# jilljenn/TF-recomm

Measured on AMD Instinct MI355X. Metric: training ratings/sec + val RMSE, MovieLens-1M SVD dim=64 @1 GPU, higher is better.
Workload: dtype f32

## Files before the change

### include/tfrecomm.h

```cpp
#ifndef TFRECOMM_H
#define TFRECOMM_H

#include <stdint.h>

#ifdef __cplusplus
extern "C" {
#endif

#define TFR_ABI_VERSION 3

typedef struct tfr_model tfr_model;

typedef enum {
    TFR_OK = 0,
    TFR_ERR_ARG = -1,
    TFR_ERR_OOB = -2,
    TFR_ERR_HIP = -3,
    TFR_ERR_STATE = -4,
    TFR_ERR_NOMEM = -5
} tfr_status;

enum {
    TFR_MU = 0,
    TFR_BU = 1,
// ... 233 lines not shown
int tfr_neighbours_dev(tfr_model* m, int32_t which, int32_t metric, const int32_t* d_rows, int64_t n, int32_t k,
                       const int64_t* d_excl_indptr, const int32_t* d_excl, int64_t lo, int64_t hi,
                       int32_t* d_ids_out, float* d_scores_out);
int tfr_svdpp_neighbours(tfr_svdpp* m, int32_t which, int32_t metric, const int32_t* rows, int64_t n, int32_t k,
                         const int64_t* excl_indptr, const int32_t* excl, int64_t lo, int64_t hi,
                         int32_t* ids_out, float* scores_out);
int tfr_svdpp_neighbours_dev(tfr_svdpp* m, int32_t which, int32_t metric, const int32_t* d_rows, int64_t n, int32_t k,
                             const int64_t* d_excl_indptr, const int32_t* d_excl, int64_t lo, int64_t hi,
                             int32_t* d_ids_out, float* d_scores_out);
int tfr_fm_neighbours(tfr_fm* m, int32_t metric, const int32_t* features, int64_t n, int32_t k,
                      const int64_t* excl_indptr, const int32_t* excl, int64_t lo, int64_t hi,
                      int32_t* ids_out, float* scores_out);
int tfr_neighbours_plan(int32_t dim, int32_t k, int64_t n, int64_t n_candidates,
                        int64_t* lds_bytes, int32_t* rows_per_block, int32_t* slices, int64_t* row_chunk);

enum {
    TFR_K_FORWARD = 0,
    TFR_K_SORT = 1,
    TFR_K_REDUCE_ITEM = 2,
    TFR_K_REDUCE_USER = 3,
    TFR_K_APPLY = 4,
    TFR_K_FINALIZE = 5,
    TFR_K_GATHER = 6,
    TFR_K_DRAW = 7,
    TFR_K_COUNT = 8
};
int tfr_profile(tfr_model* m, int32_t enable);
int tfr_kernel_plan(tfr_model* m, int64_t batch, char* buf, int64_t buflen);
int tfr_profile_read(tfr_model* m, int32_t kernel, double* total_ms, int64_t* launches);

int tfr_lds_bytes(int32_t kernel, int32_t dim, int64_t batch, int64_t user_num, int64_t item_num,
                  int64_t* static_bytes, int64_t* dynamic_bytes);

int tfr_sync(tfr_model* m);
const char* tfr_last_error(void);
int tfr_version(void);
int tfr_device_count(void);
int tfr_device_copy_rate(int32_t device, int64_t bytes, int32_t reps, double* best_gbs, double* mean_gbs);

#ifdef __cplusplus
}
#endif
#endif
```

### tf-recomm_amd/_lib.py

```python
from __future__ import annotations

import ctypes as C
import os

import numpy as np

_HERE = os.path.dirname(os.path.abspath(__file__))
LIB_PATH = os.path.join(_HERE, "csrc", "libtfrecomm_hip.so")

ABI_VERSION = 3
OK, ERR_ARG, ERR_OOB, ERR_HIP, ERR_STATE, ERR_NOMEM = 0, -1, -2, -3, -4, -5
MU, BU, BI, P, Q = 0, 1, 2, 3, 4
Y = 5
SLOT_M, SLOT_V = 8, 16
LOSS = {"mse": 0, "nll": 1}
OPTIMIZER = {"adam": 0, "sgd": 1}
ADAM_MODE = {"tf1": 0, "lazy": 1}
K_FORWARD, K_SORT, K_REDUCE_ITEM, K_REDUCE_USER, K_APPLY, K_FINALIZE, K_GATHER, K_DRAW = range(8)
NB_ITEMS, NB_USERS = 0, 1
NB_METRIC = {"dot": 0, "cosine": 1}
KERNEL_NAMES = ["forward", "sort", "reduce_item", "reduce_user", "apply", "finalize", "gather", "draw"]


class TfrOpts(C.Structure):
# ... 83 lines not shown
    "tfr_staged_ids_devptr": (C.c_int, [_p, C.POINTER(_p), _i64p]),
    "tfr_fm_create": (C.c_int, [C.POINTER(_p), C.c_int64, C.c_int32, C.POINTER(TfrOpts)]),
    "tfr_fm_destroy": (C.c_int, [_p]),
    "tfr_fm_set": (C.c_int, [_p, C.c_float, _f32p, _f32p]),
    "tfr_fm_get": (C.c_int, [_p, _f32p, _f32p, _f32p]),
    "tfr_fm_get_table": (C.c_int, [_p, C.c_int32, _f32p, C.c_int64]),
    "tfr_fm_get_step": (C.c_int, [_p, _i64p, _f32p, _f32p]),
    "tfr_fm_train_step": (C.c_int, [_p, _i64p, _i32p, _f32p, _f32p, C.c_int64, _f32p, _f32p]),
    "tfr_fm_train_step_dev": (C.c_int, [_p, _p, _p, _p, _p, C.c_int64, C.c_int64, _p]),
    "tfr_fm_init": (C.c_int, [_p, C.c_uint64, C.c_float]),
    "tfr_fm_forward": (C.c_int, [_p, _i64p, _i32p, _f32p, C.c_int64, _f32p]),
    "tfr_fm_forward_dev": (C.c_int, [_p, _p, _p, _p, C.c_int64, _p]),
    "tfr_fm_sync": (C.c_int, [_p, _f32p]),
    "tfr_fm_last_error": (C.c_char_p, []),
    "tfr_fm_upload_rows": (C.c_int, [_p, C.c_int32, _i64p, _i32p, _f32p, _f32p, C.c_int64]),
    "tfr_fm_train_steps_resident": (C.c_int, [_p, _i64p, C.c_int64, C.c_int32, _f32p]),
    "tfr_fm_gather_rows": (C.c_int, [_p, C.c_int32, _i64p, C.c_int64, _i64p, _i32p, _f32p, _f32p, C.c_int64]),
    "tfr_fm_predict_resident": (C.c_int, [_p, C.c_int32, _f32p]),
    "tfr_fm_eval_binary_resident": (C.c_int, [_p, _i64p, _f64p, _f64p, _i64p]),
    "tfr_als_create": (C.c_int, [C.POINTER(_p), C.c_int64, C.c_int64, C.c_int32, C.c_double, C.c_int32]),
    "tfr_als_destroy": (C.c_int, [_p]),
    "tfr_als_set": (C.c_int, [_p, _f64p, _f64p, _f64p, _f64p]),
    "tfr_als_get": (C.c_int, [_p, _f64p, _f64p, _f64p, _f64p, _f64p]),
    "tfr_als_set_bias": (C.c_int, [_p, C.c_double]),
    "tfr_als_load": (C.c_int, [_p, _i64p, _i64p, _f64p, C.c_int64]),
    "tfr_als_sweep": (C.c_int, [_p, C.c_int32, _f32p]),
    "tfr_als_predict": (C.c_int, [_p, _i64p, _i64p, C.c_int64, _f64p]),
    "tfr_als_last_error": (C.c_char_p, []),
    "tfr_sort_segments": (C.c_int, [_p, C.c_int32, _i32p, C.c_int64, _i32p, _i32p]),
    "tfr_kernel_plan": (C.c_int, [_p, C.c_int64, C.c_char_p, C.c_int64]),
    "tfr_profile": (C.c_int, [_p, C.c_int32]),
    "tfr_profile_read": (C.c_int, [_p, C.c_int32, C.POINTER(C.c_double), _i64p]),
    "tfr_lds_bytes": (C.c_int, [C.c_int32, C.c_int32, C.c_int64, C.c_int64, C.c_int64, _i64p, _i64p]),
    "tfr_topk": (C.c_int, [_p, _i32p, C.c_int64, C.c_int32, _i64p, _i32p, _i32p, _f32p]),
    "tfr_topk_dev": (C.c_int, [_p, _p, C.c_int64, C.c_int32, _p, _p, _p, _p]),
    "tfr_fm_topk": (C.c_int, [_p, _i32p, C.c_int64, C.c_int64, C.c_int64, C.c_int32, _i64p, _i32p, _i32p, _f32p]),
    "tfr_topk_plan": (C.c_int, [C.c_int32, C.c_int32, C.c_int64, C.c_int64, _i64p, _i32p, _i32p, _i64p]),
    "tfr_neighbours": (C.c_int, [_p, C.c_int32, C.c_int32, _i32p, C.c_int64, C.c_int32, _i64p, _i32p, C.c_int64, C.c_int64,
                                 _i32p, _f32p]),
    "tfr_neighbours_dev": (C.c_int, [_p, C.c_int32, C.c_int32, _p, C.c_int64, C.c_int32, _p, _p, C.c_int64, C.c_int64, _p, _p]),
    "tfr_svdpp_neighbours": (C.c_int, [_p, C.c_int32, C.c_int32, _i32p, C.c_int64, C.c_int32, _i64p, _i32p, C.c_int64,
                                       C.c_int64, _i32p, _f32p]),
    "tfr_svdpp_neighbours_dev": (C.c_int, [_p, C.c_int32, C.c_int32, _p, C.c_int64, C.c_int32, _p, _p, C.c_int64, C.c_int64,
                                           _p, _p]),
    "tfr_fm_neighbours": (C.c_int, [_p, C.c_int32, _i32p, C.c_int64, C.c_int32, _i64p, _i32p, C.c_int64, C.c_int64, _i32p,
                                    _f32p]),
    "tfr_neighbours_plan": (C.c_int, [C.c_int32, C.c_int32, C.c_int64, C.c_int64, _i64p, _i32p, _i32p, _i64p]),
    "tfr_rank_items": (C.c_int, [_p, _i32p, C.c_int64, _i64p, _i32p, _i64p, _i32p, _i32p]),
    "tfr_fm_rank_items": (C.c_int, [_p, _i32p, C.c_int64, C.c_int64, C.c_int64, _i64p, _i32p, _i64p, _i32p, _i32p]),
    "tfr_rank_plan": (C.c_int, [C.c_int32, C.c_int64, C.c_int64, C.c_int64, _i64p, _i32p, _i32p, _i32p, _i64p]),
    "tfr_finetune_users": (C.c_int, [_p, C.c_int64, _i32p, _i64p, _i32p, _f32p, _i64p, _i32p, _i32p, _i64p, C.c_int32,
                                     _f32p, _f32p, _f32p]),
    "tfr_finetune_plan": (C.c_int, [C.c_int32, C.c_int64, _i64p, _i32p, _i32p]),
    "tfr_svdpp_create": (C.c_int, [C.POINTER(_p), C.c_int64, C.c_int64, C.c_int32, C.POINTER(TfrOpts)]),
    "tfr_svdpp_destroy": (C.c_int, [_p]),
    "tfr_svdpp_set_table": (C.c_int, [_p, C.c_int32, _f32p, C.c_int64]),
    "tfr_svdpp_get_table": (C.c_int, [_p, C.c_int32, _f32p, C.c_int64]),
    "tfr_svdpp_init": (C.c_int, [_p, C.c_uint64, C.c_float, C.c_float]),
    "tfr_svdpp_set_implicit": (C.c_int, [_p, _i64p, _i32p]),
    "tfr_svdpp_set_frozen": (C.c_int, [_p, C.c_uint32]),
    "tfr_svdpp_set_hyper": (C.c_int, [_p, C.c_float, C.c_float]),
    "tfr_svdpp_get_step": (C.c_int, [_p, _i64p, _f32p, _f32p]),
    "tfr_svdpp_set_step": (C.c_int, [_p, C.c_int64, C.c_float, C.c_float]),
    "tfr_svdpp_forward": (C.c_int, [_p, _i32p, _i32p, C.c_int64, _f32p]),
    "tfr_svdpp_forward_dev": (C.c_int, [_p, _p, _p, C.c_int64, _p]),
    "tfr_svdpp_eval": (C.c_int, [_p, _i32p, _i32p, _f32p, C.c_int64, _f64p, _i64p]),
# ... 87 lines not shown
```

### tf-recomm_amd/csrc/api.hip

```cpp
#include <hip/hip_runtime.h>
#include <utility>
#include <stdarg.h>
#include <stdio.h>
#include <string.h>
#include <stdlib.h>
#include <math.h>
#include <new>
#include <chrono>
#include <vector>
#include <algorithm>
#include "tfrecomm.h"
#include "svd_kernels.h"
#include "topk.h"
#include "neighbours.h"
#include "rank.h"
#include "finetune.h"
#include "devbuf.h"

using namespace tfr;

static thread_local char g_err[512] = "";

static int fail(int code, const char* fmt, ...) {
    va_list ap;
// ... 2040 lines not shown

int tfr_lds_bytes(int32_t kernel, int32_t dim, int64_t batch, int64_t user_num, int64_t item_num,
                  int64_t* static_bytes, int64_t* dynamic_bytes) {
    int G, VEC;
    if (!geometry(dim, &G, &VEC)) return fail(TFR_ERR_ARG, "unsupported dim %d", dim);
    if (batch < 1 || user_num < 1 || item_num < 1) return fail(TFR_ERR_ARG, "lds_bytes: batch and row counts must be >= 1");
    const int bu = bits_for(user_num), bi = bits_for(item_num);
    const int nbmax = 1 << (bu > bi ? bu : bi);
    int64_t st = 0, dy = 0;
    if (kernel == 0 || kernel == 2) {
        if (nbmax > CSORT_MAX_BINS || !csort_eligible(batch, bu, bi)) return fail(TFR_ERR_ARG, "shape does not take the counting-sort path");
        const int64_t ntiles = (batch + CSORT_TILE - 1) / CSORT_TILE;
        if (kernel == 0) {
            if (ntiles > 16) return fail(TFR_ERR_ARG, "batch beyond 16 tiles does not take k_tile_step");
            const int epg = tile_step_epg((int)ntiles, G, VEC);
            st = (int64_t)tile_step_static_lds(G, epg);
            dy = (int64_t)tile_step_dyn_lds(G, VEC, epg, nbmax);
        } else {
            st = 256 * 4 + 16 * 64 * 4 + 16 * 3 * 4;
            dy = (int64_t)nbmax * 4;
        }
    } else if (kernel == 1 || kernel == 4) {
        st = (int64_t)seg_reduce_static_lds(G, VEC, kernel == 1);
    } else if (kernel == 3) {
        st = 2 * 624 * 4 + 2 * 10 * 4;
    } else {
        return fail(TFR_ERR_ARG, "lds_bytes: kernel must be 0 (k_tile_step), 1 (k_seg_reduce fwd), 2 (k_front), 3 (k_mt_draw), 4 (k_seg_reduce)");
    }
    if (static_bytes) *static_bytes = st;
    if (dynamic_bytes) *dynamic_bytes = dy;
    return TFR_OK;
}

static int ensure_ring(tfr_model* m, int64_t B) {
    if (B <= m->ring_cap) return TFR_OK;
    const int64_t cap = pow2_cap(B);
    m->ring_cap = 0;
    HIPCHK(m->d_ring.reserve(cap * tfr_model::HRING, m->stream));
    HIPCHK(m->h_ring.reserve(cap * tfr_model::HRING, m->stream));
    for (int z = 0; z < tfr_model::HRING; ++z)
        if (!m->ring_ev[z]) HIPCHK(hipEventCreateWithFlags(&m->ring_ev[z], hipEventDisableTiming));
    m->ring_cap = cap;
    return TFR_OK;
}

int tfr_train_step_ids(tfr_model* m, const int64_t* ids, int64_t B) {
    MODEL_ENTER(m);
    if (!m->N) return fail(TFR_ERR_STATE, "no resident triples: call tfr_upload_triples first");
    if (B < 1 || !ids) return fail(TFR_ERR_ARG, "bad batch / null ids");
    int rc;
    if ((rc = ensure_capacity(m, B))) return rc;
    if ((rc = ensure_ring(m, B))) return rc;
    const int z = m->ring_pos;
    m->ring_pos = (z + 1) % tfr_model::HRING;
    HIPCHK(hipEventSynchronize(m->ring_ev[z]));
    int64_t* h = m->h_ring + (size_t)z * m->ring_cap;
    int64_t* d = m->d_ring + (size_t)z * m->ring_cap;
    memcpy(h, ids, (size_t)B * 8);
    HIPCHK(hipMemcpyAsync(d, h, (size_t)B * 8, hipMemcpyHostToDevice, m->stream));
    HIPCHK(hipEventRecord(m->ring_ev[z], m->stream));
    m->pf_valid = false;
    return run_train_step(m, m->d_u, m->d_i, m->d_r, B, nullptr, nullptr, d, nullptr);
}

int tfr_forward_resident(tfr_model* m, int64_t lo, int64_t hi, float* logits_out) {
    MODEL_ENTER(m);
// ... 1227 lines not shown
```

### tf-recomm_amd/csrc/svd_kernels.h

```cpp
#pragma once
#include <hip/hip_runtime.h>
#include <stdint.h>

namespace tfr {

enum { MODE_INFER = 0, MODE_TRAIN = 1, MODE_EVAL = 2 };
enum { RMODE_SCRATCH = 0, RMODE_ADAM = 1, RMODE_SGD = 2 };


struct FwdArgs {
    const float* P; const float* Q; const float* bu; const float* bi; const float* mu;
    const int32_t* u; const int32_t* it; const float* r;
    const int64_t* ids; const int4* store;
    int32_t* u_out; int32_t* it_out;
    float* logits; float* g; float* partials; int32_t* err;
    int64_t B, U, I, N;
    int32_t D, loss, item_abs, reg_bias, lds_reduce;
    const int32_t* dB; int32_t qstride, bistride;
};

struct GatherArgs {
    const int64_t* ids;
    int64_t lo, B, N;
    const int4* store;
// ... 81 lines not shown
struct FinArgs {
    const float* partials; int32_t nblk;
    float* scalars; float* out;
    float* mu; float* mu_m; float* mu_v; const int32_t* err;
    int32_t update_mu, opt, clear_partials;
    int32_t out_err;
    float alpha, b1, b2, eps, lr;
};

struct ApplyPair { ApplyArgs a[2]; FinArgs f = {}; int32_t with_fin = 0; };

struct DenseArgs {
    int32_t* map; const int32_t* ks; const float* grad_rows; const float* grad_bias;
    float* dense_grad; float* dense_gbias;
    float* w; float* m; float* v; float* bias_w; float* bias_m; float* bias_v;
    const int32_t* err;
    int64_t rows, B;
    int32_t D, frozen_rows, frozen_bias, opt;
    float alpha, b1, b2, eps, lr;
};

struct DensePair { DenseArgs a[2]; FinArgs f; };


enum : int32_t {
    TFR_WT_ROWS = 1,
    TFR_WT_MOMENTS = 2,
    TFR_WT_BIAS = 4,
    TFR_WT_PIECES = 8,
    TFR_WT_PUBLISH = 16,
};
constexpr int32_t TFR_WT_DEFAULT = TFR_WT_ROWS | TFR_WT_MOMENTS | TFR_WT_BIAS | TFR_WT_PIECES | TFR_WT_PUBLISH;
int tile_step_wt();

struct TileDenseArgs {
    const int32_t* tab;
    const float* grad_rows; const float* grad_bias;
    float* w; float* m; float* v; float* bias_w; float* bias_m; float* bias_v;
    float* out_rows; float* out_bias;
    const int32_t* err;
    int64_t rows;
    int32_t D, nbins, ntiles, frozen_rows, frozen_bias, opt, skip_untouched;
    float alpha, b1, b2, eps, lr;
};
struct TileDenseLaunch { TileDenseArgs a[2]; FinArgs f; int32_t with_fin; int32_t wt; };
void launch_dense_tiles(const TileDenseLaunch& L, bool write, bool with_fin, int G, int VEC, hipStream_t s);

struct CSortArgs {
    const int32_t* keys[2];
    int32_t* ks[2]; int32_t* ps[2];
    int32_t* lrank[2];
    int32_t* hist[2];
    int32_t* offs[2];
    int32_t* binbase[2];
    int32_t* blocktot[2];
    int32_t nbins[2];
    int32_t ntiles;
    int64_t B;
};

struct FmArgs {
    const float* V; const float* W; const float* mu;
    const int64_t* indptr; const int32_t* indices; const float* data;
    float* out; int32_t* err;
    const float* y; float* s_rows; int4* ent; float* partials;
    int64_t n_rows, F;
    int32_t D, loss;
    float lam;
    int32_t variant;
};
int fm_grid(int64_t n_rows, int G, bool train);
void launch_fm(const FmArgs& a, bool train, int G, int VEC, int grid, hipStream_t s);

struct FrontArgs {
    FwdArgs f; CSortArgs c;
    int32_t* key_out[2];
    int32_t nfwd;
    int32_t tile_local;
};
// ... 131 lines not shown
```

### tf-recomm_amd/csrc/svd_kernels.hip

```cpp
#include <hip/hip_runtime.h>
#include <cstdlib>
#include <stdint.h>
#include "svd_kernels.h"
#include "finalize.inc.h"

namespace tfr {

template <int VEC> struct Frag { float v[VEC]; };

typedef float floatx4 __attribute__((ext_vector_type(4)));

template <int VEC, bool NT = false>
__device__ __forceinline__ Frag<VEC> load_frag(const float* __restrict__ row, int d0, int D) {
    Frag<VEC> f;
    if constexpr (VEC == 4) {
        if (d0 < D) {
            floatx4 t;
            if constexpr (NT) t = __builtin_nontemporal_load(reinterpret_cast<const floatx4*>(row + d0));
            else t = *reinterpret_cast<const floatx4*>(row + d0);
            f.v[0] = t.x; f.v[1] = t.y; f.v[2] = t.z; f.v[3] = t.w;
        } else {
            f.v[0] = f.v[1] = f.v[2] = f.v[3] = 0.f;
        }
    } else {
// ... 40 lines not shown
        if constexpr (VEC == 4) {
            floatx4 t; t.x = f.v[0]; t.y = f.v[1]; t.z = f.v[2]; t.w = f.v[3];
            __builtin_nontemporal_store(t, reinterpret_cast<floatx4*>(row + d0));
        } else {
            __builtin_nontemporal_store(f.v[0], row + d0);
        }
    }
}

__device__ __forceinline__ __amdgpu_buffer_rsrc_t wt_rsrc(const void* base) {
    return __builtin_amdgcn_make_buffer_rsrc(const_cast<void*>(base), 0, 0x7fffffff, 0x00020000);
}
template <int VEC>
__device__ __forceinline__ void store_frag_wt(__amdgpu_buffer_rsrc_t r, size_t off, int d0, int D, const Frag<VEC>& f) {
    if (d0 < D) {
        if constexpr (VEC == 4) {
            typedef unsigned uintx4 __attribute__((ext_vector_type(4)));
            uintx4 t;
            t.x = __float_as_uint(f.v[0]); t.y = __float_as_uint(f.v[1]); t.z = __float_as_uint(f.v[2]); t.w = __float_as_uint(f.v[3]);
            __builtin_amdgcn_raw_buffer_store_b128(t, r, (int)((off + d0) * 4), 0, 16);
        } else {
            __builtin_amdgcn_raw_buffer_store_b32(__float_as_uint(f.v[0]), r, (int)((off + d0) * 4), 0, 16);
        }
    }
}
template <int VEC>
__device__ __forceinline__ void store_frag_p(float* base, size_t off, int d0, int D, const Frag<VEC>& f, bool wt) {
    if (wt) store_frag_wt<VEC>(wt_rsrc(base), off, d0, D, f);
    else store_frag<VEC>(base + off, d0, D, f);
}
__device__ __forceinline__ void store_word_p(void* base, size_t idx, uint32_t x, bool wt) {
    if (wt) __builtin_amdgcn_raw_buffer_store_b32(x, wt_rsrc(base), (int)(idx * 4), 0, 16);
    else reinterpret_cast<uint32_t*>(base)[idx] = x;
}

template <int G>
__device__ __forceinline__ float group_sum(float x) {
#pragma unroll
    for (int o = G / 2; o >= 1; o >>= 1) x += __shfl_xor(x, o, 64);
    return x;
}

template <int G>
__device__ __forceinline__ float group_sum_lds(float x, float* wave_slot , int lane) {
    wave_slot[lane] = x;
    __builtin_amdgcn_s_waitcnt(0xc07f);
    const int g0 = lane & ~(G - 1);
    float s = 0.f;
#pragma unroll
    for (int q = 0; q < G; q += 4) {
        const float4 v = *reinterpret_cast<const float4*>(wave_slot + g0 + q);
        s += (v.x + v.y) + (v.z + v.w);
    }
    return s;
}

__device__ __forceinline__ float wave_sum(float x) {
#pragma unroll
    for (int o = 32; o >= 1; o >>= 1) x += __shfl_down(x, o, 64);
    return x;
}

template <int NV, int NW>
__device__ __forceinline__ void block_sum_store(float (&val)[NV], float* out) {
    __shared__ float red[NW][NV];
    const int lane = threadIdx.x & 63, wave = threadIdx.x >> 6;
// ... 1275 lines not shown
        } else if (slot) {
            gr = run_total<VEC, PIECE>(a.grad_rows, a.grad_bias, a.ks, a.B, (int64_t)slot - 1, (int32_t)row, d0, D, gb);
            if (gl == 0) a.map[row] = 0;
        } else {
#pragma unroll
            for (int q = 0; q < VEC; ++q) gr.v[q] = 0.f;
        }
        if (!a.frozen_rows) {
            if (a.opt == 0) {
#pragma unroll
                for (int q = 0; q < VEC; ++q) adam_sparse(w.v[q], mrow.v[q], vrow.v[q], gr.v[q], c);
                store_frag<VEC>(a.m + roff, d0, D, mrow);
                store_frag<VEC>(a.v + roff, d0, D, vrow);
            } else {
#pragma unroll
                for (int q = 0; q < VEC; ++q) w.v[q] = w.v[q] - a.lr * gr.v[q];
            }
            store_frag<VEC>(a.w + roff, d0, D, w);
        }
        if (gl == 0 && !a.frozen_bias) {
            if (a.opt == 0) {
                adam_sparse(bw, mb, vb, gb, c);
                a.bias_m[row] = mb;
                a.bias_v[row] = vb;
            } else {
                bw = bw - a.lr * gb;
            }
            a.bias_w[row] = bw;
        }
    }
}

template <int G, int VEC, bool WRITE, int NT>
__global__ __launch_bounds__(256) void k_dense_tiles(TileDenseLaunch L) {
    warm_args(L.a[blockIdx.y]);
    if (blockIdx.x == gridDim.x - 1) {
        if (blockIdx.y == 0 && L.with_fin) finalize_body(L.f);
        return;
    }
    const TileDenseArgs& a = L.a[blockIdx.y];
    const int32_t err = *a.err;
    constexpr int GPB = 256 / G;
    constexpr int EPB = 1024 / G;
    const int gl = threadIdx.x % G;
    const int d0 = gl * VEC;
    const int D = a.D;
    const AdamC c = {a.alpha, a.b1, a.b2, a.eps, 1.f - a.b1, 1.f - a.b2};
    for (int64_t row = (int64_t)blockIdx.x * GPB + threadIdx.x / G; row < a.rows;
         row += (int64_t)(gridDim.x - 1) * GPB) {
        const size_t roff = (size_t)row * D;
        Frag<VEC> w, mrow, vrow;
#pragma unroll
        for (int q = 0; q < VEC; ++q) { w.v[q] = 0.f; mrow.v[q] = 0.f; vrow.v[q] = 0.f; }
        float bw = 0.f, mb = 0.f, vb = 0.f;
        if constexpr (!WRITE) {
            if (!a.frozen_rows) {
                w = load_frag<VEC>(a.w + roff, d0, D);
                if (a.opt == 0) {
                    mrow = load_frag<VEC>(a.m + roff, d0, D);
                    vrow = load_frag<VEC>(a.v + roff, d0, D);
                }
            }
            if (gl == 0 && !a.frozen_bias) {
                bw = a.bias_w[row];
                if (a.opt == 0) { mb = a.bias_m[row]; vb = a.bias_v[row]; }
            }
        }
        Frag<VEC> tot;
#pragma unroll
        for (int q = 0; q < VEC; ++q) tot.v[q] = 0.f;
        float gb = 0.f;
// ... 323 lines not shown
        else if (fwd && rmode == RMODE_ADAM && !lean) hipLaunchKernelGGL((k_seg_reduce<g, v, RMODE_ADAM, true, false>), grid, dim3(1024), 0, s, p); \
        else if (fwd && rmode == RMODE_ADAM) hipLaunchKernelGGL((k_seg_reduce<g, v, RMODE_ADAM, true>), grid, dim3(1024), 0, s, p); \
        else if (fwd && rmode == RMODE_SCRATCH) hipLaunchKernelGGL((k_seg_reduce<g, v, RMODE_SCRATCH, true>), grid, dim3(1024), 0, s, p); \
        else if (fwd) hipLaunchKernelGGL((k_seg_reduce<g, v, RMODE_SGD, true>), grid, dim3(1024), 0, s, p); \
        else if (rmode == RMODE_SCRATCH) hipLaunchKernelGGL((k_seg_reduce<g, v, RMODE_SCRATCH>), grid, dim3(1024), 0, s, p); \
        else if (rmode == RMODE_ADAM) hipLaunchKernelGGL((k_seg_reduce<g, v, RMODE_ADAM>), grid, dim3(1024), 0, s, p);  \
        else hipLaunchKernelGGL((k_seg_reduce<g, v, RMODE_SGD>), grid, dim3(1024), 0, s, p);           \
        return;                                                                                        \
    }
    TFR_RED_CASE(4, 4) TFR_RED_CASE(8, 4) TFR_RED_CASE(16, 4) TFR_RED_CASE(32, 4) TFR_RED_CASE(64, 4)
    TFR_RED_CASE(4, 1) TFR_RED_CASE(8, 1) TFR_RED_CASE(16, 1) TFR_RED_CASE(32, 1) TFR_RED_CASE(64, 1)
#undef TFR_RED_CASE
}

void launch_apply_rows(const ApplyPair& p, int n, int opt, int G, int VEC, hipStream_t s) {
    int64_t B = p.a[0].B;
    if (n > 1 && p.a[1].B > B) B = p.a[1].B;
    bool all_split = p.a[0].only_split != 0;
    if (n > 1 && !p.a[1].only_split) all_split = false;
    if (all_split) B = (B + 1024 / G - 1) / (1024 / G);
    const dim3 grid(entry_grid(B, G) + (p.with_fin ? 1 : 0), n);
#define TFR_APP_CASE(g, v)                                                                  \
    if (G == g && VEC == v) {                                                               \
        if (opt == 0) hipLaunchKernelGGL((k_apply_rows<g, v, 0>), grid, dim3(256), 0, s, p); \
        else if (opt == 1) hipLaunchKernelGGL((k_apply_rows<g, v, 1>), grid, dim3(256), 0, s, p); \
        else hipLaunchKernelGGL((k_apply_rows<g, v, 2>), grid, dim3(256), 0, s, p);         \
        return;                                                                             \
    }
    TFR_APP_CASE(4, 4) TFR_APP_CASE(8, 4) TFR_APP_CASE(16, 4) TFR_APP_CASE(32, 4) TFR_APP_CASE(64, 4)
    TFR_APP_CASE(4, 1) TFR_APP_CASE(8, 1) TFR_APP_CASE(16, 1) TFR_APP_CASE(32, 1) TFR_APP_CASE(64, 1)
#undef TFR_APP_CASE
}

void launch_dense_tiles(const TileDenseLaunch& L, bool write, bool with_fin, int G, int VEC, hipStream_t s) {
    const int gpb = 256 / G;
    int64_t rows = L.a[0].rows > L.a[1].rows ? L.a[0].rows : L.a[1].rows;
    int64_t nb = (rows + gpb - 1) / gpb;
    if (nb > 4096) nb = 4096;
    if (nb < 1) nb = 1;
    const dim3 grid((int)nb + 1, 2);
    TileDenseLaunch LL = L;
    LL.with_fin = with_fin ? 1 : 0;
    LL.wt = tile_step_wt() & (TFR_WT_ROWS | TFR_WT_MOMENTS | TFR_WT_BIAS);
#define TFR_DT_LAUNCH(g, v, wr, nt) hipLaunchKernelGGL((k_dense_tiles<g, v, wr, nt>), grid, dim3(256), 0, s, LL)
#define TFR_DT_CASE(g, v)                                                                         \
    if (G == g && VEC == v) {                                                                     \
        const int nt = L.a[0].ntiles;                                                             \
        if (write) {                                                                              \
            if (nt <= 4) TFR_DT_LAUNCH(g, v, true, 4); else if (nt <= 8) TFR_DT_LAUNCH(g, v, true, 8);      \
            else if (nt <= 10) TFR_DT_LAUNCH(g, v, true, 10);                                               \
            else if (nt <= 12) TFR_DT_LAUNCH(g, v, true, 12); else TFR_DT_LAUNCH(g, v, true, 16);           \
        } else {                                                                                  \
            if (nt <= 4) TFR_DT_LAUNCH(g, v, false, 4); else if (nt <= 8) TFR_DT_LAUNCH(g, v, false, 8);    \
            else if (nt <= 10) TFR_DT_LAUNCH(g, v, false, 10);                                              \
            else if (nt <= 12) TFR_DT_LAUNCH(g, v, false, 12); else TFR_DT_LAUNCH(g, v, false, 16);         \
        }                                                                                         \
        return;                                                                                   \
    }
    TFR_DT_CASE(4, 4) TFR_DT_CASE(8, 4) TFR_DT_CASE(16, 4) TFR_DT_CASE(32, 4) TFR_DT_CASE(64, 4)
    TFR_DT_CASE(4, 1) TFR_DT_CASE(8, 1) TFR_DT_CASE(16, 1) TFR_DT_CASE(32, 1) TFR_DT_CASE(64, 1)
#undef TFR_DT_LAUNCH
#undef TFR_DT_CASE
}

void launch_adam_dense(DensePair& p, int n, int G, int VEC, hipStream_t s, const FinArgs* fin) {
    if (fin) { p.f = *fin; n = 3; }
    const int gpb = 256 / G;
    int64_t rows = p.a[0].rows;
    if (n > 1 && p.a[1].rows > rows) rows = p.a[1].rows;
    int64_t nb = (rows + gpb - 1) / gpb;
    if (nb > 4096) nb = 4096;
    if (nb < 1) nb = 1;
    const dim3 grid((int)nb, n);
#define TFR_DEN_CASE(g, v) \
    if (G == g && VEC == v) { hipLaunchKernelGGL((k_adam_dense<g, v>), grid, dim3(256), 0, s, p); return; }
    TFR_DEN_CASE(4, 4) TFR_DEN_CASE(8, 4) TFR_DEN_CASE(16, 4) TFR_DEN_CASE(32, 4) TFR_DEN_CASE(64, 4)
    TFR_DEN_CASE(4, 1) TFR_DEN_CASE(8, 1) TFR_DEN_CASE(16, 1) TFR_DEN_CASE(32, 1) TFR_DEN_CASE(64, 1)
#undef TFR_DEN_CASE
}

static int flat_grid(int64_t n) {
    int64_t nb = (n + 255) / 256;
    if (nb > 2048) nb = 2048;
    if (nb < 1) nb = 1;
    return (int)nb;
}

void launch_gather_rows(const GatherRowsArgs& a, int G, int VEC, hipStream_t s) {
    const int gpb = 256 / G;
    int64_t nb = (a.n + gpb - 1) / gpb;
    if (nb > 8192) nb = 8192;
    if (nb < 1) nb = 1;
#define TFR_GR_CASE(g, v) \
    if (G == g && VEC == v) { hipLaunchKernelGGL((k_gather_rows<g, v>), dim3((int)nb), dim3(256), 0, s, a); return; }
    TFR_GR_CASE(4, 4) TFR_GR_CASE(8, 4) TFR_GR_CASE(16, 4) TFR_GR_CASE(32, 4) TFR_GR_CASE(64, 4)
    TFR_GR_CASE(4, 1) TFR_GR_CASE(8, 1) TFR_GR_CASE(16, 1) TFR_GR_CASE(32, 1) TFR_GR_CASE(64, 1)
// ... 58 lines not shown
```

Measured before the change: 563.0 million.

## Add row-per-thread-group dense tile sweep using buffer loads with OOB masking

Adds a new path in k_dense_tiles, on by default for VEC==4 shapes where one grid covers all rows. Each row group loads its tile entries, parameters and gradient pieces with raw buffer loads. Masked loads use an out-of-bounds offset instead of branches, and loads are batched behind sched barriers to raise memory-level parallelism. It also sets occupancy via a launch_bounds minimum-blocks hint and adds a residency query API. Extra register pressure could cause spills, and the buffer-load masking assumes 32-bit offsets.

After: 597.3 million (median of 6 runs). 6.1% higher.

```diff
diff --git a/include/tfrecomm.h b/include/tfrecomm.h
--- a/include/tfrecomm.h
+++ b/include/tfrecomm.h
@@ -289,6 +289,9 @@
 int tfr_lds_bytes(int32_t kernel, int32_t dim, int64_t batch, int64_t user_num, int64_t item_num,
                   int64_t* static_bytes, int64_t* dynamic_bytes);
 
+int tfr_sweep_residency(int32_t dim, int64_t batch, int64_t user_num, int64_t item_num,
+                        int32_t* blocks_per_cu, int64_t* scratch_bytes, int64_t* grid_blocks);
+
 int tfr_sync(tfr_model* m);
 const char* tfr_last_error(void);
 int tfr_version(void);
diff --git a/tf-recomm_amd/_lib.py b/tf-recomm_amd/_lib.py
--- a/tf-recomm_amd/_lib.py
+++ b/tf-recomm_amd/_lib.py
@@ -139,6 +139,7 @@
     "tfr_profile": (C.c_int, [_p, C.c_int32]),
     "tfr_profile_read": (C.c_int, [_p, C.c_int32, C.POINTER(C.c_double), _i64p]),
     "tfr_lds_bytes": (C.c_int, [C.c_int32, C.c_int32, C.c_int64, C.c_int64, C.c_int64, _i64p, _i64p]),
+    "tfr_sweep_residency": (C.c_int, [C.c_int32, C.c_int64, C.c_int64, C.c_int64, _i32p, _i64p, _i64p]),
     "tfr_topk": (C.c_int, [_p, _i32p, C.c_int64, C.c_int32, _i64p, _i32p, _i32p, _f32p]),
     "tfr_topk_dev": (C.c_int, [_p, _p, C.c_int64, C.c_int32, _p, _p, _p, _p]),
     "tfr_fm_topk": (C.c_int, [_p, _i32p, C.c_int64, C.c_int64, C.c_int64, C.c_int32, _i64p, _i32p, _i32p, _f32p]),
diff --git a/tf-recomm_amd/csrc/api.hip b/tf-recomm_amd/csrc/api.hip
--- a/tf-recomm_amd/csrc/api.hip
+++ b/tf-recomm_amd/csrc/api.hip
@@ -2096,6 +2096,27 @@
     return TFR_OK;
 }
 
+int tfr_sweep_residency(int32_t dim, int64_t batch, int64_t user_num, int64_t item_num,
+                        int32_t* blocks_per_cu, int64_t* scratch_bytes, int64_t* grid_blocks) {
+    int G, VEC;
+    if (!geometry(dim, &G, &VEC)) return fail(TFR_ERR_ARG, "unsupported dim %d", dim);
+    if (batch < 1 || user_num < 1 || item_num < 1) return fail(TFR_ERR_ARG, "sweep_residency: batch and row counts must be >= 1");
+    const int bu = bits_for(user_num), bi = bits_for(item_num);
+    const int64_t ntiles = (batch + CSORT_TILE - 1) / CSORT_TILE;
+    if ((1 << (bu > bi ? bu : bi)) > CSORT_MAX_BINS || !csort_eligible(batch, bu, bi) || ntiles > 16)
+        return fail(TFR_ERR_ARG, "shape does not take k_dense_tiles");
+    const void* k = dense_tiles_kernel(false, G, VEC, (int)ntiles);
+    if (!k) return fail(TFR_ERR_ARG, "no k_dense_tiles instantiation for dim %d", dim);
+    int nblk = 0;
+    hipFuncAttributes attr;
+    HIPCHK(hipOccupancyMaxActiveBlocksPerMultiprocessor(&nblk, k, 256, 0));
+    HIPCHK(hipFuncGetAttributes(&attr, k));
+    if (blocks_per_cu) *blocks_per_cu = nblk;
+    if (scratch_bytes) *scratch_bytes = (int64_t)attr.localSizeBytes;
+    if (grid_blocks) *grid_blocks = 2 * ((int64_t)dense_tiles_grid(user_num > item_num ? user_num : item_num, G) + 1);
+    return TFR_OK;
+}
+
 static int ensure_ring(tfr_model* m, int64_t B) {
     if (B <= m->ring_cap) return TFR_OK;
     const int64_t cap = pow2_cap(B);
diff --git a/tf-recomm_amd/csrc/svd_kernels.h b/tf-recomm_amd/csrc/svd_kernels.h
--- a/tf-recomm_amd/csrc/svd_kernels.h
+++ b/tf-recomm_amd/csrc/svd_kernels.h
@@ -137,6 +137,7 @@
 };
 constexpr int32_t TFR_WT_DEFAULT = TFR_WT_ROWS | TFR_WT_MOMENTS | TFR_WT_BIAS | TFR_WT_PIECES | TFR_WT_PUBLISH;
 int tile_step_wt();
+int sweep_rounds();
 
 struct TileDenseArgs {
     const int32_t* tab;
@@ -148,8 +149,11 @@
     int32_t D, nbins, ntiles, frozen_rows, frozen_bias, opt, skip_untouched;
     float alpha, b1, b2, eps, lr;
 };
-struct TileDenseLaunch { TileDenseArgs a[2]; FinArgs f; int32_t with_fin; int32_t wt; };
+struct TileDenseLaunch { TileDenseArgs a[2]; FinArgs f; int32_t with_fin; int32_t wt; int32_t rounds; };
 void launch_dense_tiles(const TileDenseLaunch& L, bool write, bool with_fin, int G, int VEC, hipStream_t s);
+const void* dense_tiles_kernel(bool write, int G, int VEC, int ntiles);
+int dense_tiles_grid(int64_t rows, int G);
+bool dense_tiles_rounds_taken(int64_t rows, int D, int G, int VEC);
 
 struct CSortArgs {
     const int32_t* keys[2];
diff --git a/tf-recomm_amd/csrc/svd_kernels.hip b/tf-recomm_amd/csrc/svd_kernels.hip
--- a/tf-recomm_amd/csrc/svd_kernels.hip
+++ b/tf-recomm_amd/csrc/svd_kernels.hip
@@ -96,6 +96,23 @@
 __device__ __forceinline__ void store_word_p(void* base, size_t idx, uint32_t x, bool wt) {
     if (wt) __builtin_amdgcn_raw_buffer_store_b32(x, wt_rsrc(base), (int)(idx * 4), 0, 16);
     else reinterpret_cast<uint32_t*>(base)[idx] = x;
+}
+
+constexpr int BUF_NONE = (int)0x80000000u;
+__device__ __forceinline__ uint32_t buf_load_word(__amdgpu_buffer_rsrc_t r, int byte_off) {
+    return __builtin_amdgcn_raw_buffer_load_b32(r, byte_off, 0, 0);
+}
+template <int VEC>
+__device__ __forceinline__ Frag<VEC> buf_load_frag(__amdgpu_buffer_rsrc_t r, int byte_off) {
+    Frag<VEC> f;
+    if constexpr (VEC == 4) {
+        typedef unsigned uintx4 __attribute__((ext_vector_type(4)));
+        const uintx4 t = __builtin_amdgcn_raw_buffer_load_b128(r, byte_off, 0, 0);
+        f.v[0] = __uint_as_float(t.x); f.v[1] = __uint_as_float(t.y); f.v[2] = __uint_as_float(t.z); f.v[3] = __uint_as_float(t.w);
+    } else {
+        f.v[0] = __uint_as_float(buf_load_word(r, byte_off));
+    }
+    return f;
 }
 
 template <int G>
@@ -1437,11 +1454,168 @@
 }
 
 template <int G, int VEC, bool WRITE, int NT>
-__global__ __launch_bounds__(256) void k_dense_tiles(TileDenseLaunch L) {
+__device__ __forceinline__ void dense_tiles_rounds(const TileDenseLaunch& L) {
+    const TileDenseArgs& a = L.a[blockIdx.y];
+    constexpr int GPB = 256 / G;
+    constexpr int EPB = 1024 / G;
+    constexpr int D = G * VEC;
+    constexpr int NB = (NT > 12) ? 8 : NT;
+    const int gl = threadIdx.x % G;
+    const int d0 = gl * VEC;
+    const int row = (int)blockIdx.x * GPB + threadIdx.x / G;
+    if (row >= a.rows) return;
+    const __amdgpu_buffer_rsrc_t rtab =
+        __builtin_amdgcn_make_buffer_rsrc(const_cast<int32_t*>(a.tab), 0, a.ntiles * a.nbins * 4, 0x00020000);
+    int32_t ent[NT];
+#pragma unroll
+    for (int t = 0; t < NT; ++t) ent[t] = (int32_t)buf_load_word(rtab, (t * a.nbins + row) * 4);
+    int32_t err = (int32_t)buf_load_word(wt_rsrc(a.err), 0);
+    __builtin_amdgcn_sched_barrier(0);
+    const int roff = (row * D + d0) * 4;
+    Frag<VEC> w, mrow, vrow;
+    float bw = 0.f, mb = 0.f, vb = 0.f;
+    if constexpr (!WRITE) {
+        const int ow = a.frozen_rows ? BUF_NONE : roff;
+        const int om = (a.frozen_rows || a.opt != 0) ? BUF_NONE : roff;
+        w = buf_load_frag<VEC>(wt_rsrc(a.w), ow);
+        mrow = buf_load_frag<VEC>(wt_rsrc(a.m), om);
+        vrow = buf_load_frag<VEC>(wt_rsrc(a.v), om);
+        const int ob = (gl == 0 && !a.frozen_bias) ? row * 4 : BUF_NONE;
+        const int obm = (gl == 0 && !a.frozen_bias && a.opt == 0) ? row * 4 : BUF_NONE;
+        bw = __uint_as_float(buf_load_word(wt_rsrc(a.bias_w), ob));
+        mb = __uint_as_float(buf_load_word(wt_rsrc(a.bias_m), obm));
+        vb = __uint_as_float(buf_load_word(wt_rsrc(a.bias_v), obm));
+    }
+    __builtin_amdgcn_sched_barrier(0);
+    asm volatile("" : "+v"(err) : : "memory");
+    if (err) return;
+    int s0 = -1, s1 = -1, nk1 = 0;
+    bool deep = false, touched = false;
+#pragma unroll
+    for (int t = 0; t < NT; ++t) {
+        const int32_t e = ent[t];
+        const int off = e & 0xffff;
+        const int pp = t * 1024 + (off / EPB + 1) * EPB;
+        const int end = t * 1024 + off + (e >> 16);
+        const bool has1 = pp < end;
+        deep = deep || pp + EPB < end;
+        s1 = (has1 && nk1 == 1) ? pp : s1;
+        s0 = (has1 && nk1 == 0) ? pp : s0;
+        nk1 += has1 ? 1 : 0;
+        touched = touched || (e >> 16);
+    }
+    const __amdgpu_buffer_rsrc_t rg = wt_rsrc(a.grad_rows), rgb = wt_rsrc(a.grad_bias);
+    Frag<VEC> tot, c0, c1;
+#pragma unroll
+    for (int q = 0; q < VEC; ++q) tot.v[q] = 0.f;
+    float gb = 0.f, cb0 = 0.f, cb1 = 0.f;
+#pragma unroll
+    for (int t0 = 0; t0 < NT; t0 += NB) {
+        Frag<VEC> x[NB];
+        float xb[NB];
+#pragma unroll
+        for (int t = 0; t < NB; ++t) {
+            const int32_t e = ent[t0 + t];
+            const int j = (t0 + t) * 1024 + (e & 0xffff);
+            x[t] = buf_load_frag<VEC>(rg, (e >> 16) ? (j * D + d0) * 4 : BUF_NONE);
+            xb[t] = __uint_as_float(buf_load_word(rgb, ((e >> 16) && gl == 0) ? j * 4 : BUF_NONE));
+        }
+        if (t0 == 0) {
+            c0 = buf_load_frag<VEC>(rg, s0 >= 0 ? (s0 * D + d0) * 4 : BUF_NONE);
+            cb0 = __uint_as_float(buf_load_word(rgb, (s0 >= 0 && gl == 0) ? s0 * 4 : BUF_NONE));
+            c1 = buf_load_frag<VEC>(rg, s1 >= 0 ? (s1 * D + d0) * 4 : BUF_NONE);
+            cb1 = __uint_as_float(buf_load_word(rgb, (s1 >= 0 && gl == 0) ? s1 * 4 : BUF_NONE));
+        }
+        __builtin_amdgcn_sched_barrier(0);
+#pragma unroll
+        for (int t = 0; t < NB; ++t) {
+#pragma unroll
+            for (int q = 0; q < VEC; ++q) tot.v[q] += x[t].v[q];
+            gb += xb[t];
+        }
+    }
+    if (nk1 <= 2 && !deep) {
+#pragma unroll
+        for (int q = 0; q < VEC; ++q) tot.v[q] += c0.v[q];
+        gb += cb0;
+#pragma unroll
+        for (int q = 0; q < VEC; ++q) tot.v[q] += c1.v[q];
+        gb += cb1;
+    } else {
+        for (int k = 1;; ++k) {
+            bool more = false;
+#pragma unroll
+            for (int t0 = 0; t0 < NT; t0 += NB) {
+                Frag<VEC> y[NB];
+                float yb[NB];
+#pragma unroll
+                for (int t = 0; t < NB; ++t) {
+                    const int32_t e = ent[t0 + t];
+                    const int j = (t0 + t) * 1024 + (e & 0xffff);
+                    const int pp = (j / EPB + k) * EPB;
+                    const bool has = pp < j + (e >> 16);
+                    y[t] = buf_load_frag<VEC>(rg, has ? (pp * D + d0) * 4 : BUF_NONE);
+                    yb[t] = __uint_as_float(buf_load_word(rgb, (has && gl == 0) ? pp * 4 : BUF_NONE));
+                    more = more || has;
+                }
+#pragma unroll
+                for (int t = 0; t < NB; ++t) {
+#pragma unroll
+                    for (int q = 0; q < VEC; ++q) tot.v[q] += y[t].v[q];
+                    gb += yb[t];
+                }
+            }
+            if (!more) break;
+        }
+    }
+    const size_t rfl = (size_t)row * D;
+    if constexpr (WRITE) {
+        if (touched) {
+            store_frag<VEC>(a.out_rows + rfl, d0, D, tot);
+            if (gl == 0) a.out_bias[row] = gb;
+        }
+    } else {
+        if (!touched && a.skip_untouched) return;
+        const AdamC c = {a.alpha, a.b1, a.b2, a.eps, 1.f - a.b1, 1.f - a.b2};
+        const int wt = L.wt;
+        if (!a.frozen_rows) {
+            if (a.opt == 0) {
+#pragma unroll
+                for (int q = 0; q < VEC; ++q) adam_sparse(w.v[q], mrow.v[q], vrow.v[q], tot.v[q], c);
+                store_frag_p<VEC>(a.m, rfl, d0, D, mrow, wt & TFR_WT_MOMENTS);
+                store_frag_p<VEC>(a.v, rfl, d0, D, vrow, wt & TFR_WT_MOMENTS);
+            } else {
+#pragma unroll
+                for (int q = 0; q < VEC; ++q) w.v[q] = __builtin_fmaf(-a.lr, tot.v[q], w.v[q]);
+            }
+            store_frag_p<VEC>(a.w, rfl, d0, D, w, wt & TFR_WT_ROWS);
+        }
+        if (gl == 0 && !a.frozen_bias) {
+            const bool wb = wt & TFR_WT_BIAS;
+            if (a.opt == 0) {
+                adam_sparse(bw, mb, vb, gb, c);
+                store_word_p(a.bias_m, (size_t)row, __float_as_uint(mb), wb);
+                store_word_p(a.bias_v, (size_t)row, __float_as_uint(vb), wb);
+            } else {
+                bw = bw - __fmul_rn(a.lr, gb);
+            }
+            store_word_p(a.bias_w, (size_t)row, __float_as_uint(bw), wb);
+        }
+    }
+}
+
+template <int G, int VEC, bool WRITE, int NT>
+__global__ __launch_bounds__(256, (NT > 12 && VEC == 4 && !WRITE) ? 2 : 3) void k_dense_tiles(TileDenseLaunch L) {
     warm_args(L.a[blockIdx.y]);
     if (blockIdx.x == gridDim.x - 1) {
         if (blockIdx.y == 0 && L.with_fin) finalize_body(L.f);
         return;
+    }
+    if constexpr (VEC == 4) {
+        if (L.rounds) {
+            dense_tiles_rounds<G, VEC, WRITE, NT>(L);
+            return;
+        }
     }
     const TileDenseArgs& a = L.a[blockIdx.y];
     const int32_t err = *a.err;
@@ -1831,36 +2005,63 @@
 #undef TFR_APP_CASE
 }
 
-void launch_dense_tiles(const TileDenseLaunch& L, bool write, bool with_fin, int G, int VEC, hipStream_t s) {
+int sweep_rounds() {
+    static int on = -1;
+    if (on < 0) { const char* e = getenv("TFR_SWEEP_ROUNDS"); on = (e && e[0] == '0') ? 0 : 1; }
+    return on;
+}
+
+int dense_tiles_grid(int64_t rows, int G) {
     const int gpb = 256 / G;
-    int64_t rows = L.a[0].rows > L.a[1].rows ? L.a[0].rows : L.a[1].rows;
     int64_t nb = (rows + gpb - 1) / gpb;
     if (nb > 4096) nb = 4096;
     if (nb < 1) nb = 1;
-    const dim3 grid((int)nb + 1, 2);
+    return (int)nb;
+}
+
+bool dense_tiles_rounds_taken(int64_t rows, int D, int G, int VEC) {
+    return sweep_rounds() && VEC == 4 && D == G * VEC && rows <= (int64_t)dense_tiles_grid(rows, G) * (256 / G);
+}
+
+#define TFR_DT_PICK(g, v, wr, nt) TFR_DT_DO((k_dense_tiles<g, v, wr, nt>))
+#define TFR_DT_CASE(g, v)                                                                         \
+    if (G == g && VEC == v) {                                                                     \
+        if (write) {                                                                              \
+            if (nt <= 4) TFR_DT_PICK(g, v, true, 4); else if (nt <= 8) TFR_DT_PICK(g, v, true, 8);          \
+            else if (nt <= 10) TFR_DT_PICK(g, v, true, 10);                                                 \
+            else if (nt <= 12) TFR_DT_PICK(g, v, true, 12); else TFR_DT_PICK(g, v, true, 16);               \
+        } else {                                                                                  \
+            if (nt <= 4) TFR_DT_PICK(g, v, false, 4); else if (nt <= 8) TFR_DT_PICK(g, v, false, 8);        \
+            else if (nt <= 10) TFR_DT_PICK(g, v, false, 10);                                                \
+            else if (nt <= 12) TFR_DT_PICK(g, v, false, 12); else TFR_DT_PICK(g, v, false, 16);             \
+        }                                                                                         \
+    }
+#define TFR_DT_ALL                                                                                \
+    TFR_DT_CASE(4, 4) TFR_DT_CASE(8, 4) TFR_DT_CASE(16, 4) TFR_DT_CASE(32, 4) TFR_DT_CASE(64, 4)  \
+    TFR_DT_CASE(4, 1) TFR_DT_CASE(8, 1) TFR_DT_CASE(16, 1) TFR_DT_CASE(32, 1) TFR_DT_CASE(64, 1)
+
+const void* dense_tiles_kernel(bool write, int G, int VEC, int nt) {
+#define TFR_DT_DO(k) return reinterpret_cast<const void*>(&k)
+    TFR_DT_ALL
+#undef TFR_DT_DO
+    return nullptr;
+}
+
+void launch_dense_tiles(const TileDenseLaunch& L, bool write, bool with_fin, int G, int VEC, hipStream_t s) {
+    const int64_t rows = L.a[0].rows > L.a[1].rows ? L.a[0].rows : L.a[1].rows;
+    const dim3 grid(dense_tiles_grid(rows, G) + 1, 2);
     TileDenseLaunch LL = L;
     LL.with_fin = with_fin ? 1 : 0;
     LL.wt = tile_step_wt() & (TFR_WT_ROWS | TFR_WT_MOMENTS | TFR_WT_BIAS);
-#define TFR_DT_LAUNCH(g, v, wr, nt) hipLaunchKernelGGL((k_dense_tiles<g, v, wr, nt>), grid, dim3(256), 0, s, LL)
-#define TFR_DT_CASE(g, v)                                                                         \
-    if (G == g && VEC == v) {                                                                     \
-        const int nt = L.a[0].ntiles;                                                             \
-        if (write) {                                                                              \
-            if (nt <= 4) TFR_DT_LAUNCH(g, v, true, 4); else if (nt <= 8) TFR_DT_LAUNCH(g, v, true, 8);      \
-            else if (nt <= 10) TFR_DT_LAUNCH(g, v, true, 10);                                               \
-            else if (nt <= 12) TFR_DT_LAUNCH(g, v, true, 12); else TFR_DT_LAUNCH(g, v, true, 16);           \
-        } else {                                                                                  \
-            if (nt <= 4) TFR_DT_LAUNCH(g, v, false, 4); else if (nt <= 8) TFR_DT_LAUNCH(g, v, false, 8);    \
-            else if (nt <= 10) TFR_DT_LAUNCH(g, v, false, 10);                                              \
-            else if (nt <= 12) TFR_DT_LAUNCH(g, v, false, 12); else TFR_DT_LAUNCH(g, v, false, 16);         \
-        }                                                                                         \
-        return;                                                                                   \
-    }
-    TFR_DT_CASE(4, 4) TFR_DT_CASE(8, 4) TFR_DT_CASE(16, 4) TFR_DT_CASE(32, 4) TFR_DT_CASE(64, 4)
-    TFR_DT_CASE(4, 1) TFR_DT_CASE(8, 1) TFR_DT_CASE(16, 1) TFR_DT_CASE(32, 1) TFR_DT_CASE(64, 1)
-#undef TFR_DT_LAUNCH
+    LL.rounds = (L.a[0].D == L.a[1].D && dense_tiles_rounds_taken(rows, L.a[0].D, G, VEC)) ? 1 : 0;
+    const int nt = L.a[0].ntiles;
+#define TFR_DT_DO(k) do { hipLaunchKernelGGL(k, grid, dim3(256), 0, s, LL); return; } while (0)
+    TFR_DT_ALL
+#undef TFR_DT_DO
+}
+#undef TFR_DT_ALL
 #undef TFR_DT_CASE
-}
+#undef TFR_DT_PICK
 
 void launch_adam_dense(DensePair& p, int n, int G, int VEC, hipStream_t s, const FinArgs* fin) {
     if (fin) { p.f = *fin; n = 3; }
```
